# JianCao92/speaker-diarization

Hardware: AMD Instinct MI355X
Metric: diarized audio throughput (CD gw/BIC + CL hi/BIC) (higher is better)
Workload: dtype f64

## Files before the change

speaker-diarization_amd/csrc/spkd_cluster.hpp:

```cpp
#pragma once
#include "spkd_device.hpp"
#include "spkd_quad.hpp"
#include "spkd_tri.hpp"
#include "../../include/spkd.h"

namespace spkd {

constexpr double MAXINT_F = 9223372036854775808.0;
constexpr double PEN_UNIT = 39.0 + 0.5 * 39.0 * 40.0;
constexpr int AUX = 3 * DA;
constexpr int ERR_DEGENERATE_MERGE = 2;

__device__ __forceinline__ unsigned long long dkey(double v) {
    unsigned long long b = (unsigned long long)__double_as_longlong(v);
    return (b >> 63) ? ~b : (b | 0x8000000000000000ull);
}
__device__ __forceinline__ double dkey_inv(unsigned long long k) {
    unsigned long long b = (k >> 63) ? (k & 0x7fffffffffffffffull) : ~k;
    return __longlong_as_double((long long)b);
}
template <bool MAXOP>
__device__ __forceinline__ unsigned wave_red_u32(unsigned x) {
    auto op = [](unsigned a, unsigned b) { return MAXOP ? (a > b ? a : b) : (a < b ? a : b); };
    x = op(x, (unsigned)__builtin_amdgcn_update_dpp((int)x, (int)x, 0xB1, 0xf, 0xf, false));
// ... 556 lines not shown
    r.mc = okey != ~0ull ? (int)oc : NO_COL;
    r.nc = __any(nc != NO_COL) ? (int)wave_red_u32<false>((unsigned)nc) : NO_COL;
    return r;
}

__device__ __forceinline__ bool row_cache_after_merge(int variant, double d, int sa, int sb,
                                                      double& rm, int& ra, int& rn) {
    if (variant != 1) return ra == sb || rn == sb;
    const bool nan_hit = rn == sa || rn == sb;
    if (ra == sa || ra == sb || nan_hit) {
        if (nan_hit || !(d < rm)) return true;
        rm = d; ra = sa;
    } else if (d != d) {
        if (sa < rn) rn = sa;
    } else if (d < rm || (d == rm && sa < ra)) {
        rm = d; ra = sa;
    }
    return false;
}

template <class Alive>
__device__ __forceinline__ double final_matrix_max(const double* __restrict__ Dm, long long N, Alive alive,
                                                   double* s_tmax, int tid) {
    const int lane = tid & (WAVE - 1), wave = tid >> 6;
    double tmax = -__builtin_huge_val();
    bool anynan = false;
    for (long long r = wave; r < N; r += AHC_WAVES) {
        if (!alive(r)) continue;
        const double* row = Dm + r * N;
        for (long long c = lane; c < N; c += WAVE) {
            if (!alive(c)) continue;
            const double v = row[c];
            if (v != v) anynan = true; else tmax = v > tmax ? v : tmax;
        }
    }
#pragma unroll
    for (int s = 1; s < WAVE; s <<= 1) {
        const double t2 = __shfl_xor(tmax, s);
        tmax = t2 > tmax ? t2 : tmax;
    }
    anynan = __any(anynan);
    if (lane == 0) s_tmax[wave] = anynan ? __builtin_nan("") : tmax;
    __syncthreads();
    double mx = s_tmax[0];
    if (tid == 0) {
        for (int w = 1; w < AHC_WAVES; ++w) {
            const double x = s_tmax[w];
            if (mx == mx) mx = (x != x) ? x : (x > mx ? x : mx);
        }
    }
    return mx;
}

__device__ __forceinline__ void refresh_rows(const double* __restrict__ Dm, long long N,
                                             const int32_t* __restrict__ al, int32_t* __restrict__ dirty,
                                             double* __restrict__ rmin, int32_t* __restrict__ rarg,
                                             int32_t* __restrict__ rnan, unsigned long long* masks,
                                             int tid, int wave, int lane) {
    const long long n_chunks = (N + WAVE - 1) / WAVE;
    for (long long ch = wave; ch < n_chunks; ch += AHC_WAVES) {
        const long long rl = ch * WAVE + lane;
        const long long rc = rl < N ? rl : N - 1;
        const int fa = al[rc], fd = dirty[rc];
        const unsigned long long mk = __ballot(rl < N && fa && fd);
        if (lane == 0) masks[ch] = mk;
    }
    __syncthreads();
    int ord = 0;
    for (long long ch = 0; ch < n_chunks; ++ch) {
        const long long r0 = ch * WAVE;
        unsigned long long todo = masks[ch];
        while (todo) {
            const int b = __builtin_ctzll(todo);
            todo &= todo - 1;
            if ((ord++ & (AHC_WAVES - 1)) != wave) continue;
            const long long r = r0 + b;
            const RowMin e = scan_row(Dm + r * N, N, [&](long long c) { return al[c] != 0; }, -1, 0.0, lane);
            if (lane == 0) { rmin[r] = e.mv; rarg[r] = e.mc; rnan[r] = e.nc; dirty[r] = 0; }
#ifdef SPKD_PROFILE
            if (lane == 0) atomicAdd(&g_ahc_prof[0], 1ull);
#endif
        }
    }
}

template <bool TWO>
__global__ __launch_bounds__(AHC_TPB) void k_ahc(
        double* __restrict__ ex, double* __restrict__ pk, const int64_t* __restrict__ seg_off,
        int variant, int kind, int max_spk, double lambdac, double threshold,
        double* __restrict__ ld, double* __restrict__ aux,
        double* __restrict__ mat, const int64_t* __restrict__ mat_off,
        int32_t* __restrict__ alive, double* __restrict__ tmp,
        double* __restrict__ rmin_all, int32_t* __restrict__ rcache_all,
        int32_t* __restrict__ out_n, int32_t* __restrict__ out_a, int32_t* __restrict__ out_b,
        double* __restrict__ out_d, unsigned long long* stat_max, unsigned long long* stat_min,
        double* __restrict__ final_max, double* __restrict__ final_min, int* err,
        double* pinv_ws) {
    extern __shared__ int32_t ids[];
    __shared__ double ldsA[QREC];
    __shared__ unsigned long long red3[AHC_WAVES][3];
    __shared__ unsigned long long s_masks[AHC_MAX_N / WAVE];
    __shared__ int s_cnt[2];
    __shared__ int s_nids;
    __shared__ int s_next;
    __shared__ double s_tmax[AHC_WAVES];
    const int tid = threadIdx.x, lane = lane_id(), wave = tid >> 6;
    const QuadLane L = quad_lane();
    const int p = blockIdx.x;
    const int64_t off = seg_off[p];
    const long long N = seg_off[p + 1] - off;
    double* Dm = mat + mat_off[p];
    int32_t* al = alive + off;
    double* ldp = ld + off;
    double* tp = tmp + off;
    double* rmin = rmin_all + off;
    int32_t* rarg = rcache_all + 3 * off;
    int32_t* rnan = rarg + N;
    int32_t* dirty = rnan + N;
    for (long long c = tid; c < N; c += AHC_TPB) { al[c] = 1; dirty[c] = 1; }
    __syncthreads();
    long long m = N;
    int n_merges = 0;
    const long long INF_IDX = 0x7fffffffffffffffLL;
    double fmin = 0.0;
#ifdef SPKD_PROFILE
    unsigned long long ahc_acc[5] = {0ull, 0ull, 0ull, 0ull, 0ull}, ahc_t = clock64();
#define AHC_TICK(i) do { const unsigned long long now_ = clock64(); ahc_acc[i] += now_ - ahc_t; ahc_t = now_; } while (0)
#else
#define AHC_TICK(i) ((void)0)
#endif
    while (true) {
        refresh_rows(Dm, N, al, dirty, rmin, rarg, rnan, s_masks, tid, wave, lane);
        __syncthreads();
        AHC_TICK(0);
        unsigned long long kb = ~0ull, ib = ~0ull, inan = ~0ull;
        for (long long r = tid; r < N; r += AHC_TPB) {
            if (!al[r]) continue;
            const double v = rmin[r];
            const int c = rarg[r], nc = rnan[r];
            if (nc != NO_COL) { const unsigned long long l = (unsigned long long)(r * N + nc); inan = l < inan ? l : inan; }
            if (c != NO_COL) {
                const unsigned long long kv = dkey(v);
                if (kv < kb) { kb = kv; ib = (unsigned long long)(r * N + c); }
            }
        }
        {
            const unsigned long long wk = wave_red_u64<false>(kb);
            const unsigned long long wi = wave_red_u64<false>(kb == wk ? ib : ~0ull);
            const unsigned long long wn = __any(inan != ~0ull) ? wave_red_u64<false>(inan) : ~0ull;
            if (lane == 0) { red3[wave][0] = wk; red3[wave][1] = wi; red3[wave][2] = wn; }
        }
        __syncthreads();
        unsigned long long bk = red3[0][0], bi = red3[0][1], bn = red3[0][2];
#pragma unroll
        for (int w = 1; w < AHC_WAVES; ++w) {
            const unsigned long long ok = red3[w][0], oi = red3[w][1], on = red3[w][2];
            const bool t = ok < bk || (ok == bk && oi < bi);
            bk = t ? ok : bk; bi = t ? oi : bi;
            bn = on < bn ? on : bn;
        }
        const bool has_nan = bn != ~0ull;
        const double mind = has_nan ? __builtin_nan("") : (bi != ~0ull ? dkey_inv(bk) : __builtin_huge_val());
        const long long index = has_nan ? (long long)bn : (bi != ~0ull ? (long long)bi : INF_IDX);
        fmin = mind;
        const bool go = (mind <= threshold) || (max_spk > 0 && m > max_spk);
        if (!go) break;
        AHC_TICK(1);
        const long long r0 = index / N, c0 = index - r0 * N;
        if (r0 == c0) {
            if (tid == 0) atomicOr(err, ERR_DEGENERATE_MERGE);
            break;
        }
        const long long sa = r0 < c0 ? r0 : c0, sb = r0 < c0 ? c0 : r0;
        if (tid < 2) s_cnt[tid] = 0;
        if (tid == 0) { s_nids = 1; s_next = 0; }
        __syncthreads();
        {
            int ca = 0, cb = 0;
            for (long long c = tid; c < sb; c += AHC_TPB) {
                if (al[c]) { cb++; if (c < sa) ca++; }
            }
            ca = __builtin_amdgcn_readlane(wave_scan_i32(ca), WAVE - 1);
            cb = __builtin_amdgcn_readlane(wave_scan_i32(cb), WAVE - 1);
            if (lane == 0 && ca) atomicAdd(&s_cnt[0], ca);
            if (lane == 0 && cb) atomicAdd(&s_cnt[1], cb);
        }
        __syncthreads();
        if (tid == 0) {
            const int64_t o = off + n_merges;
            out_a[o] = s_cnt[0]; out_b[o] = s_cnt[1]; out_d[o] = mind;
            al[sb] = 0;
            ids[0] = (int32_t)sa;
        }
        n_merges++;
        m--;
#ifdef SPKD_PROFILE
        if (tid == 0) atomicAdd(&g_ahc_prof[1], 1ull);
#endif
        double* A = ex + (off + sa) * QREC;
        const double* B = ex + (off + sb) * QREC;
        {
            double* Ap = pk + (off + sa) * REC;
            const double* Bp = pk + (off + sb) * REC;
            constexpr int NQ = (QREC + AHC_TPB - 1) / AHC_TPB, NP = (REC + AHC_TPB - 1) / AHC_TPB;
            double qa[NQ], qb[NQ], pa[NP], pb[NP];
#pragma unroll
            for (int u = 0; u < NQ; ++u) {
                const int e = tid + u * AHC_TPB;
                qa[u] = A[e < QREC ? e : 0]; qb[u] = B[e < QREC ? e : 0];
            }
#pragma unroll
            for (int u = 0; u < NP; ++u) {
                const int e = tid + u * AHC_TPB;
                pa[u] = Ap[e < REC ? e : 0]; pb[u] = Bp[e < REC ? e : 0];
            }
#pragma unroll
            for (int u = 0; u < NQ; ++u) {
                const int e = tid + u * AHC_TPB;
                const double v = qa[u] + qb[u];
                if (e < QREC) { A[e] = v; ldsA[e] = v; }
            }
#pragma unroll
            for (int u = 0; u < NP; ++u) {
                const int e = tid + u * AHC_TPB;
                if (e < REC) Ap[e] = pa[u] + pb[u];
            }
        }
        __syncthreads();
        for (long long c0 = 0; c0 < N; c0 += AHC_TPB) {
            const long long c = c0 + tid;
            const bool take = c < N && c != sa && al[c < N ? c : N - 1];
            const unsigned long long mk = __ballot(take);
            int base = 0;
            if (lane == 0 && mk) base = atomicAdd(&s_nids, __popcll(mk));
            base = __shfl(base, 0);
            if (take) ids[base + __popcll(mk & ((1ull << lane) - 1ull))] = (int32_t)c;
        }
        __syncthreads();
        AHC_TICK(2);
        const int nids = s_nids;
        const double nA = ldsA[QREC_COUNT_AT];
        if (kind == SPKD_KL2) {
            if (wave == 0) kl2_aux_from_qr(ldsA, aux + (off + sa) * AUX, pinv_ws);
        } else {
            for (;;) {
                int q4 = 0;
                if (lane == 0) q4 = atomicAdd(&s_next, 1);
                const int base = 4 * __builtin_amdgcn_readfirstlane(q4);
                if (base >= nids) break;
                int k = base + L.m;
                const bool valid = k < nids;
                k = valid ? k : nids - 1;
                const int32_t slot = ids[k];
                const double v = quad_pair_det<TWO>(kind, ldsA, nA, A, ex + (off + slot) * QREC, pk + (off + slot) * REC, k == 0, L, err);
                if (valid && L.t == 0) {
                    if (k == 0) ldp[sa] = log(v); else tp[slot] = v;
                }
            }
        }
        __syncthreads();
        AHC_TICK(3);
        double wmax = __builtin_nan(""), wmin = __builtin_nan("");
        const double ldA = ldp[sa];
        for (long long c = tid; c < N; c += AHC_TPB) {
            if (c == sa || !al[c]) continue;
            double d;
            if (kind == SPKD_KL2) {
                d = kl2_from_aux_serial(aux + (off + sa) * AUX, aux + (off + c) * AUX);
            } else {
                const double nC = qr_count(ex + (off + c) * QREC);
                d = finish_distance(kind, lambdac, nA, ldA, nC, ldp[c], log(tp[c]));
            }
            Dm[sa * N + c] = d;
            const double rm0 = rmin[c];
            const int ra0 = rarg[c], rn0 = rnan[c];
            double rm = rm0;
            int ra = ra0, rn = rn0;
            if (variant == 1) Dm[c * N + sa] = d;
            if (row_cache_after_merge(variant, d, (int)sa, (int)sb, rm, ra, rn)) dirty[c] = 1;
            else {
                if (rm != rm0 || ra != ra0) { rmin[c] = rm; rarg[c] = ra; }
                if (rn != rn0) rnan[c] = rn;
            }
            if (variant == 1 && stat_valid(d)) {
                wmax = (wmax != wmax || d > wmax) ? d : wmax;
                wmin = (wmin != wmin || d < wmin) ? d : wmin;
            }
        }
        if (tid == 0) dirty[sa] = 1;
        if (variant == 1) {
            const unsigned long long kmax = wave_red_u64<true>(wmax == wmax ? dkey(wmax) : 0ull);
            const unsigned long long kmin = wave_red_u64<false>(wmin == wmin ? dkey(wmin) : ~0ull);
            if (lane == 0) {
                if (kmax != 0ull) atomicMax(stat_max + p, kmax);
                if (kmin != ~0ull) atomicMin(stat_min + p, kmin);
            }
        }
        __syncthreads();
        AHC_TICK(4);
    }
#ifdef SPKD_PROFILE
    if (tid == 0) for (int i = 0; i < 5; ++i) atomicAdd(&g_ahc_prof[2 + i], ahc_acc[i]);
#endif
    const double mx = final_matrix_max(Dm, N, [&](long long c) { return al[c] != 0; }, s_tmax, tid);
    if (tid == 0) {
        out_n[p] = n_merges;
        final_max[p] = mx;
        final_min[p] = fmin;
    }
}

constexpr int STEP_WAVES = 4;
constexpr int STEP_WIDE_FROM = 1024;
constexpr int STEP_PARTNERS = 4 * STEP_WAVES - 1;
constexpr int ALIVE_ROUND = 0x7fffffff;
constexpr int STEP_MAX_N = 16384;
constexpr int STEP_IDX_SHIFT = 14;

struct StepState {
    int32_t done, n_merges;
    long long psa;
    double fmin;
    double diag;
};

__host__ __device__ inline unsigned long long step_slot_word(int round, int new_slot, int old_slot) {
    return ((unsigned long long)(unsigned)round << 40) | ((unsigned long long)(unsigned)new_slot << 20) |
           (unsigned long long)(unsigned)old_slot;
}
__device__ __forceinline__ int step_slot_of(unsigned long long w, int k) {
    return ((int)(w >> 40) < k) ? (int)((w >> 20) & 0xfffffull) : (int)(w & 0xfffffull);
}

struct StepSel {
    double rmin, newrow;
    int32_t rarg, rnan, death, pad;
};

struct StepArrays {
    double* ex;
    double* pk;
    double* exm;
    double* pkm;
    int32_t* death;
    StepSel* sel2;
    unsigned long long* sw;
    double* cnt;
    StepState* state2;
    int64_t n_total;
    int32_t n_prob;
};

__global__ __launch_bounds__(AHC_TPB) void k_step_init(
        const int64_t* __restrict__ seg_off, const double* __restrict__ mat,
        const int64_t* __restrict__ mat_off, StepArrays Q) {
    const int lane = lane_id(), wave = threadIdx.x >> 6;
    const int p = blockIdx.y;
    const int64_t off = seg_off[p];
    const long long N = seg_off[p + 1] - off;
    if (blockIdx.x == 0 && threadIdx.x == 0) {
        StepState S;
// ... 312 lines not shown
    if (kind != SPKD_KL2 && lead && tid == 0) ldp[sa] = ldA;
    {
        const int j = tid;
        bool rescan = false;
        double d = 0.0;
        if (fin) {
            const long long r = fin_r;
            if (kind == SPKD_KL2) d = kl2_from_aux_serial(s_auxA, aux + (off + r) * AUX);
            else d = finish_distance(kind, lambdac, nA, ldA, fin_nC, fin_ld, s_ldx[j]);
            double rm;
            int ra, rn;
            if (r == psa) { rm = s_psa.mv; ra = s_psa.mc; rn = s_psa.nc; }
            else { rm = fin_sel.rmin; ra = fin_sel.rarg; rn = fin_sel.rnan; }
            Dm[sa * N + r] = d;
            sel_w[r].newrow = d;
            if (variant == 1) Dm[r * N + sa] = d;
            rescan = row_cache_after_merge(variant, d, (int)sa, (int)sb, rm, ra, rn);
            if (!rescan) { sel_w[r].rmin = rm; sel_w[r].rarg = ra; sel_w[r].rnan = rn; }
        }
        if (tid < 4 * STEP_WAVES) { s_rescan[tid] = rescan ? 1 : 0; s_dfin[tid] = d; }
        __syncthreads();
        for (int jj = 1 + wave; jj <= mine_n; jj += SW) {
            if (!s_rescan[jj]) continue;
            const long long r = s_ids[first + jj - 1];
            const RowMin e = scan_row(Dm + r * N, N, [&](long long c) { return c != sb && death[c] > k; },
                                      variant == 1 ? sa : -1, s_dfin[jj], lane);
            if (lane == 0) { sel_w[r].rmin = e.mv; sel_w[r].rarg = e.mc; sel_w[r].rnan = e.nc; }
        }
    }
    STEP_TICK(6);
#ifdef SPKD_PROFILE
    if (lead && tid == 0) atomicAdd(&g_ahc_prof[1], 1ull);
#endif
    if (lead && tid == 0) {
        StepState T;
        T.done = 0; T.n_merges = n_merges + 1; T.psa = sa; T.fmin = mind; T.diag = diag_sa;
        *Snext = T;
    }
}

__global__ __launch_bounds__(AHC_TPB) void k_step_final(
        int last_round, const int64_t* __restrict__ seg_off, const double* __restrict__ mat,
        const int64_t* __restrict__ mat_off, StepArrays Q, int32_t* __restrict__ out_n,
        double* __restrict__ final_max, double* __restrict__ final_min) {
    __shared__ double s_tmax[AHC_WAVES];
    const int tid = threadIdx.x;
    const int p = blockIdx.x;
    const int64_t off = seg_off[p];
    const long long N = seg_off[p + 1] - off;
    const int32_t* death = Q.death + off;
    const StepState S = Q.state2[(size_t)((last_round + 1) & 1) * Q.n_prob + p];
    const double mx = final_matrix_max(mat + mat_off[p], N, [&](long long c) { return death[c] == ALIVE_ROUND; }, s_tmax, tid);
    if (tid == 0) {
        out_n[p] = S.n_merges;
        final_max[p] = mx;
        final_min[p] = S.fmin;
    }
}

constexpr int CIN_WAVES = 4;
constexpr int CIN_TPB = CIN_WAVES * WAVE;

struct CinKeep {
    double* dist;
    long long cap;
    long long* dist_off;
    int* status;
    long long off = 0;
    __device__ bool room(long long K) const { return off + K <= cap; }
    __device__ void refuse() const { atomicOr(status, 4); }
    __device__ double* row() const { return dist + off; }
    __device__ void step() {}
    __device__ void seen(double) {}
    __device__ void decided(long long s, long long K, double, bool lead) {
        off += K;
        if (lead) dist_off[s + 1] = off;
    }
};

struct CinSummary {
    double* dists;
    double* mind;
    double smax = __builtin_nan(""), smin = __builtin_nan("");
    double tmax = __builtin_nan(""), tmin = __builtin_nan("");
    __device__ bool room(long long) const { return true; }
    __device__ void refuse() const {}
    __device__ double* row() const { return dists; }
    __device__ void step() { tmax = tmin = __builtin_nan(""); }
    __device__ void seen(double d) {
        if (!stat_valid(d)) return;
        if (!(tmax >= d)) tmax = d;
        if (!(tmin <= d)) tmin = d;
    }
    __device__ void decided(long long s, long long, double m, bool lead) {
        if (!lead) return;
        mind[s] = m;
        if (tmax == tmax && !(smax >= tmax)) smax = tmax;
        if (tmin == tmin && !(smin <= tmin)) smin = tmin;
    }
};

template <bool TWO, class Out>
__device__ __forceinline__ long long cluster_in_chain(
        const double* __restrict__ seg_ex, const double* __restrict__ seg_pk, const double* __restrict__ seg_ld,
        const double* __restrict__ seg_aux, long long n, int kind, double lambdac, double threshold,
        double* __restrict__ clu_ex, double* __restrict__ clu_pk, double* __restrict__ clu_ld, double* __restrict__ clu_aux,
        double* __restrict__ tmp, int32_t* __restrict__ label, Out& out, long long& K, int* err,
        double* pinv_ws) {
    __shared__ double ldsA[QREC];
// ... 140 lines not shown
```

speaker-diarization_amd/csrc/spkd_hip.hip:

```cpp
#include <hip/hip_runtime.h>

#include <algorithm>
#include <cmath>
#include <cstddef>
#include <cstdio>
#include <cstdlib>
#include <cstring>
#include <string>
#include <atomic>
#include <thread>
#include <vector>

#include "../../include/spkd.h"
#include "spkd_cd.hpp"
#include "spkd_cluster.hpp"
#include "spkd_device.hpp"
#include "spkd_handoff.hpp"
#include "spkd_stats.hpp"
#include "spkd_mfcc.hpp"
#include "spkd_vad.hpp"

using namespace spkd;

namespace {
constexpr int N_SLOTS = 40;
enum { PIN_GW_TURNS = 0, PIN_GW_LINES, PIN_AHC_OUT, N_PIN };
}

struct spkd_ctx {
    int device = 0;
    hipStream_t stream = nullptr;
    bool own_stream = false;
    bool gw_lds_ok = false;
    int gw_waves = 0;
    unsigned long long init_keys[2] = {0ull, ~0ull};
    int step_waves = 0;
    int step_partners = 0;
    int64_t last_gw_items = 0;
    std::string err;
    int* d_err = nullptr;
    unsigned long long* d_counter = nullptr;
    hipEvent_t ev0 = nullptr, ev1 = nullptr;
    float last_ms = 0.f;
    hipEvent_t ka[SPKD_N_TIMERS] = {}, kb[SPKD_N_TIMERS] = {};
    bool kused[SPKD_N_TIMERS] = {};
    float kms[SPKD_N_TIMERS] = {};
    void* slot[N_SLOTS] = {};
    size_t slot_bytes[N_SLOTS] = {};
    void* pinv_ws = nullptr;
    double* pinv_cur = nullptr;
    void* pin[N_PIN] = {};
    size_t pin_bytes[N_PIN] = {};
    std::vector<int64_t> redo_line, redo_begin, redo_end;
    std::vector<Chunk> redo_chunks;
    std::vector<int64_t> redo_setoff;
    std::vector<int32_t> redo_sets;
};

namespace {

spkd_status fail(spkd_ctx* c, spkd_status s, const std::string& msg) {
    if (c) c->err = msg;
    return s;
}

#define HIPCHK(c, call)                                                              \
    do {                                                                             \
        hipError_t e_ = (call);                                                      \
        if (e_ != hipSuccess)                                                        \
            return fail((c), SPKD_EHIP, std::string(#call) + ": " + hipGetErrorString(e_)); \
    } while (0)

#define TRY(expr) do { const spkd_status s_ = (expr); if (s_ != SPKD_OK) return s_; } while (0)

spkd_status scratch(spkd_ctx* c, int slot, size_t bytes, void** out) {
    if (bytes == 0) bytes = 16;
    if (c->slot_bytes[slot] < bytes) {
        if (c->slot[slot]) HIPCHK(c, hipFree(c->slot[slot]));
        c->slot[slot] = nullptr;
        c->slot_bytes[slot] = 0;
        size_t want = bytes + bytes / 4;
        hipError_t e = hipMalloc(&c->slot[slot], want);
        if (e != hipSuccess) {
            want = bytes;
            e = hipMalloc(&c->slot[slot], want);
        }
        if (e != hipSuccess) return fail(c, SPKD_ENOMEM, "scratch allocation failed");
        c->slot_bytes[slot] = want;
    }
    *out = c->slot[slot];
// ... 122 lines not shown
    spkd_ctx* const c;
    const int idx;
    Timer(spkd_ctx* ctx, int i) : c(ctx), idx(i) { (void)hipEventRecord(c->ka[idx], c->stream); }
    ~Timer() { (void)hipEventRecord(c->kb[idx], c->stream); c->kused[idx] = true; }
};

enum {
    S_CHUNKS = 0, S_SETOFF, S_PARTIAL, S_IDXA, S_IDXB, S_TERMS, S_TURNS, S_SNAP, S_CAND,
    S_GW_N_WIN, S_GW_WIN_DET, S_GW_WIN_MAXD, S_GW_DET_START, S_GW_DET_MAXI, S_GW_DET_D, S_GW_FINAL_START, S_LOG,
    S_AHC_STATS, S_AHC_LD, S_AHC_AUX, S_AHC_MAT, S_AHC_MISC, S_AHC_OUT, S_AHC_OFF, S_AHC_PROB, S_AHC_PACKED, S_MFCC_TAB, S_MFCC_STATIC,
    S_STEP_EXM, S_STEP_PKM, S_STEP_MISC, S_GMM_TAB, S_GMM_IDX,
    S_CP_TURNS, S_CP_TIMES, S_CP_LINES, S_REDO_STATS, S_REDO_IDX, S_COUNT
};
static_assert(S_COUNT <= N_SLOTS, "scratch slot table too small");

}

extern "C" {

int spkd_abi_version(void) { return SPKD_ABI_VERSION; }

static spkd_status create_ctx(int device, void* stream, bool borrow, spkd_ctx** out) {
    if (!out) return SPKD_EINVAL;
    *out = nullptr;
    int count = 0;
    if (hipGetDeviceCount(&count) != hipSuccess || device < 0 || device >= count) return SPKD_EHIP;
    spkd_ctx* c = new spkd_ctx();
    c->device = device;
    if (hipSetDevice(device) != hipSuccess) { delete c; return SPKD_EHIP; }
    if (borrow) {
        c->stream = (hipStream_t)stream;
    } else {
        if (hipStreamCreateWithFlags(&c->stream, hipStreamDefault) != hipSuccess) { delete c; return SPKD_EHIP; }
        c->own_stream = true;
    }
    if (hipMalloc(&c->d_err, sizeof(int)) != hipSuccess ||
        hipMalloc(&c->d_counter, 2 * sizeof(unsigned long long)) != hipSuccess ||
        hipEventCreate(&c->ev0) != hipSuccess || hipEventCreate(&c->ev1) != hipSuccess) {
        spkd_destroy(c);
        return SPKD_EHIP;
    }
    for (int i = 0; i < SPKD_N_TIMERS; ++i)
        if (hipEventCreate(&c->ka[i]) != hipSuccess || hipEventCreate(&c->kb[i]) != hipSuccess) {
            spkd_destroy(c);
            return SPKD_EHIP;
        }
    int lds_max = 0;
    c->gw_lds_ok = hipDeviceGetAttribute(&lds_max, hipDeviceAttributeMaxSharedMemoryPerBlock, device) == hipSuccess &&
                   Gw<4>::LDS_BYTES <= lds_max &&
                   hipFuncSetAttribute((const void*)k_gw<8>, hipFuncAttributeMaxDynamicSharedMemorySize, Gw<8>::LDS_BYTES) == hipSuccess &&
                   hipFuncSetAttribute((const void*)k_gw<4>, hipFuncAttributeMaxDynamicSharedMemorySize, Gw<4>::LDS_BYTES) == hipSuccess &&
                   hipFuncSetAttribute((const void*)k_gw<2>, hipFuncAttributeMaxDynamicSharedMemorySize, Gw<2>::LDS_BYTES) == hipSuccess &&
                   hipFuncSetAttribute((const void*)k_gw<1>, hipFuncAttributeMaxDynamicSharedMemorySize, Gw<1>::LDS_BYTES) == hipSuccess;
    if (const char* e = getenv("SPKD_GW_WAVES")) c->gw_waves = atoi(e);
    if (const char* e = getenv("SPKD_STEP_WAVES")) { const int v = atoi(e); c->step_waves = (v == 4 || v == 8) ? v : 0; }
    if (const char* e = getenv("SPKD_STEP_PARTNERS")) { const int v = atoi(e); c->step_partners = (v == 3 || v == 7 || v == 15) ? v : 0; }
    *out = c;
    return SPKD_OK;
}

spkd_status spkd_create(int device, void* stream, spkd_ctx** out) {
    return create_ctx(device, stream, stream != nullptr, out);
}

spkd_status spkd_create_on_stream(int device, void* stream, spkd_ctx** out) {
    return create_ctx(device, stream, true, out);
}

void spkd_destroy(spkd_ctx* c) {
    if (!c) return;
    (void)hipSetDevice(c->device);
    if (c->stream) (void)hipStreamSynchronize(c->stream);
    for (int i = 0; i < N_SLOTS; ++i)
        if (c->slot[i]) (void)hipFree(c->slot[i]);
    if (c->d_err) (void)hipFree(c->d_err);
    if (c->pinv_ws) (void)hipFree(c->pinv_ws);
    for (int i = 0; i < N_PIN; ++i)
        if (c->pin[i]) (void)hipHostFree(c->pin[i]);
    if (c->d_counter) (void)hipFree(c->d_counter);
    if (c->ev0) (void)hipEventDestroy(c->ev0);
    if (c->ev1) (void)hipEventDestroy(c->ev1);
    for (int i = 0; i < SPKD_N_TIMERS; ++i) {
        if (c->ka[i]) (void)hipEventDestroy(c->ka[i]);
        if (c->kb[i]) (void)hipEventDestroy(c->kb[i]);
    }
    if (c->own_stream && c->stream) (void)hipStreamDestroy(c->stream);
    delete c;
}

const char* spkd_last_error(const spkd_ctx* c) { return c ? c->err.c_str() : "null context"; }

spkd_status spkd_sync(spkd_ctx* c) {
    if (!c) return SPKD_EINVAL;
    HIPCHK(c, hipStreamSynchronize(c->stream));
    return SPKD_OK;
}

spkd_status spkd_malloc(spkd_ctx* c, size_t bytes, void** d_ptr) {
    if (!c || !d_ptr) return SPKD_EINVAL;
    HIPCHK(c, hipSetDevice(c->device));
    hipError_t e = hipMalloc(d_ptr, bytes ? bytes : 16);
    if (e != hipSuccess) return fail(c, SPKD_ENOMEM, hipGetErrorString(e));
    return SPKD_OK;
}

spkd_status spkd_free(spkd_ctx* c, void* d_ptr) {
// ... 434 lines not shown
        h_n_done[p] = done2[2 * p];
        h_n_clusters[p] = done2[2 * p + 1];
    }
    return st;
}

spkd_status spkd_distance_rows(spkd_ctx* c, int variant, int kind, double lambdac, const double* d_stats,
                               int64_t n, int64_t row_begin, int64_t row_end, double* d_rows,
                               double* h_stat_max, double* h_stat_min) {
    if (!c || n < 0 || bad_kind(kind) || (variant != 1 && variant != 2)) return SPKD_EINVAL;
    if (row_begin < 0 || row_end < row_begin || row_end > n) return fail(c, SPKD_EINVAL, "distance_rows: bad row block");
    if (h_stat_max) *h_stat_max = std::nan("");
    if (h_stat_min) *h_stat_min = std::nan("");
    if (n == 0 || row_end == row_begin) return SPKD_OK;
    if (!d_stats || !d_rows) return fail(c, SPKD_EINVAL, "null argument");
    const int64_t seg_off[2] = {0, n};
    AhcPrep B;
    MatrixPlan plan;
    plan.row_begin = row_begin;
    plan.row_end = row_end;
    unsigned long long keys[2] = {0ull, ~0ull};
    Call call(c);
    TRY(call.opened);
    TRY(use_kind(c, kind, &kind));
    TRY(ahc_prepare(c, d_stats, seg_off, 1, variant, kind, lambdac, B, plan));
    HIPCHK(c, hipMemcpyAsync(d_rows, B.mat + row_begin * n, (size_t)(row_end - row_begin) * n * sizeof(double),
                             hipMemcpyDeviceToDevice, c->stream));
    HIPCHK(c, hipMemcpyAsync(&keys[0], B.smax, sizeof(unsigned long long), hipMemcpyDeviceToHost, c->stream));
    HIPCHK(c, hipMemcpyAsync(&keys[1], B.smin, sizeof(unsigned long long), hipMemcpyDeviceToHost, c->stream));
    const spkd_status st = call.finish();
    if (h_stat_max) *h_stat_max = key_to_double(keys[0], true);
    if (h_stat_min) *h_stat_min = key_to_double(keys[1], false);
    return st;
}

namespace {
spkd_status ahc_impl(spkd_ctx* c, const double* d_stats, const int64_t* h_seg_off, int64_t n_prob,
                     const spkd_ahc_params* P, const MatrixPlan& plan, int32_t* h_n_merges, int32_t* h_merge_a,
                     int32_t* h_merge_b, double* h_merge_d, double* h_stat_max, double* h_stat_min) {
    if (!c || !P || n_prob < 0) return SPKD_EINVAL;
    if (n_prob == 0) return SPKD_OK;
    if (!d_stats || !h_seg_off || !h_n_merges || !h_merge_a || !h_merge_b || !h_merge_d ||
        !h_stat_max || !h_stat_min)
        return fail(c, SPKD_EINVAL, "null argument");
    if ((P->variant != 1 && P->variant != 2) || bad_kind(P->kind))
        return fail(c, SPKD_EINVAL, "bad variant / kind");
    for (int64_t p = 0; p < n_prob; ++p)
        if (h_seg_off[p + 1] - h_seg_off[p] < 1) return fail(c, SPKD_EINVAL, "empty clustering problem");
    int64_t n_max = 0;
    for (int64_t p = 0; p < n_prob; ++p) n_max = std::max<int64_t>(n_max, h_seg_off[p + 1] - h_seg_off[p]);
    if (n_max > AHC_MAX_N) return fail(c, SPKD_EINVAL, "clustering problem larger than 65536 records");
    int path = P->path;
    if (path != SPKD_AHC_MONO && path != SPKD_AHC_WIDE) path = n_prob <= 64 ? SPKD_AHC_WIDE : SPKD_AHC_MONO;
    const size_t lds = (size_t)(n_max + 4) * sizeof(int32_t);
    if (path == SPKD_AHC_MONO && lds > 150 * 1024) path = SPKD_AHC_WIDE;
    if (path == SPKD_AHC_WIDE && n_max > STEP_MAX_N)
        return fail(c, SPKD_EINVAL, "clustering problem larger than 16384 records (wide merge loop)");
    AhcPrep B;
    std::vector<unsigned long long> kmax((size_t)n_prob), kmin((size_t)n_prob);
    std::vector<double> fmax((size_t)n_prob), fmin((size_t)n_prob);
    Call call(c);
    TRY(call.opened);
    spkd_ahc_params Pk;
    TRY(kernel_params(c, P, Pk));
    TRY(ahc_prepare(c, d_stats, h_seg_off, n_prob, P->variant, P->kind, P->lambdac, B, plan));
    const int64_t n_total = B.n_total;
    const size_t nt = (size_t)n_total, np = (size_t)n_prob;
    double *d_merge_d, *d_tmp, *d_rmin, *d_fmax, *d_fmin;
    int32_t *d_a, *d_b, *d_alive, *d_rcache, *d_n;
    TRY(carve(c, scratch, S_AHC_OUT, [&](Layout L) {
        return L.part(d_merge_d, nt).part(d_tmp, nt).part(d_rmin, nt).part(d_fmax, np).part(d_fmin, np)
            .part(d_a, nt).part(d_b, nt).part(d_alive, nt).part(d_rcache, 3 * nt).part(d_n, np).bytes();
    }));
    if (path == SPKD_AHC_MONO) {
        auto kahc = P->kind == SPKD_GLR ? k_ahc<true> : k_ahc<false>;
        if (lds > 48 * 1024)
            (void)hipFuncSetAttribute((const void*)kahc, hipFuncAttributeMaxDynamicSharedMemorySize, (int)lds);
        Timer t(c, SPKD_T_AHC);
        hipLaunchKernelGGL(kahc, dim3((unsigned)n_prob), dim3(AHC_TPB), lds, c->stream,
                           B.ex, B.pk, (const int64_t*)B.seg_off, P->variant, P->kind, P->max_spk, P->lambdac,
                           P->threshold, B.ld, B.aux, B.mat, (const int64_t*)B.mat_off, d_alive, d_tmp,
                           d_rmin, d_rcache, d_n, d_a, d_b, d_merge_d, B.smax, B.smin, d_fmax, d_fmin, c->d_err,
                           c->pinv_cur);
    } else {
        StepArrays Q;
        void *pe = nullptr, *pp = nullptr;
        TRY(carve(c, scratch, S_STEP_MISC, [&](Layout L) {
            return L.part(Q.sel2, 2 * nt).part(Q.cnt, nt).part(Q.sw, nt).part(Q.state2, 2 * np).part(Q.death, nt).bytes();
        }));
        TRY(scratch(c, S_STEP_EXM, nt * QREC * sizeof(double), &pe));
        TRY(scratch(c, S_STEP_PKM, nt * REC * sizeof(double), &pp));
        Q.ex = B.ex; Q.pk = B.pk; Q.exm = (double*)pe; Q.pkm = (double*)pp;
        Q.n_total = n_total;
        Q.n_prob = (int32_t)n_prob;
        const int step_waves = c->step_waves ? c->step_waves : (n_max > STEP_WIDE_FROM ? 8 : 4);
        const bool glr_k = P->kind == SPKD_GLR;
        using StepKernel = decltype(&k_ahc_step<false, 4, 3>);
        StepKernel kvar[3];
        if (step_waves == 8) {
            kvar[0] = glr_k ? k_ahc_step<true, 8, 3> : k_ahc_step<false, 8, 3>;
            kvar[1] = glr_k ? k_ahc_step<true, 8, 7> : k_ahc_step<false, 8, 7>;
            kvar[2] = glr_k ? k_ahc_step<true, 8, STEP_PARTNERS> : k_ahc_step<false, 8, STEP_PARTNERS>;
        } else {
            kvar[0] = glr_k ? k_ahc_step<true, 4, 3> : k_ahc_step<false, 4, 3>;
            kvar[1] = glr_k ? k_ahc_step<true, 4, 7> : k_ahc_step<false, 4, 7>;
            kvar[2] = glr_k ? k_ahc_step<true, 4, STEP_PARTNERS> : k_ahc_step<false, 4, STEP_PARTNERS>;
        }
        auto sp_of_round = [&](int64_t partners) -> int {
            if (c->step_partners) return c->step_partners;
            const int64_t free_cus = 255;
            if (partners * n_prob <= 3 * free_cus) return 3;
            if (partners * n_prob <= 7 * free_cus) return 7;
            return STEP_PARTNERS;
        };
        const size_t nch_max = (size_t)((n_max + WAVE - 1) / WAVE);
        const size_t step_lds = ((size_t)2 * n_max + nch_max + 2) * sizeof(int32_t) + nch_max * sizeof(unsigned long long);
        if (step_lds + 20 * 1024 > 48 * 1024)
            for (int v = 0; v < 3; ++v)
                (void)hipFuncSetAttribute((const void*)kvar[v], hipFuncAttributeMaxDynamicSharedMemorySize, (int)step_lds);
        Timer t(c, SPKD_T_AHC);
        const unsigned row_blocks = (unsigned)((n_max + AHC_WAVES - 1) / AHC_WAVES);
        hipLaunchKernelGGL(k_step_init, dim3(row_blocks, (unsigned)n_prob), dim3(AHC_TPB), 0, c->stream,
                           (const int64_t*)B.seg_off, (const double*)B.mat, (const int64_t*)B.mat_off, Q);
        for (int64_t it = 1; it < n_max; ++it) {
            const int64_t partners = n_max - it - 1;
            const int step_sp = sp_of_round(partners);
            StepKernel kstep = kvar[step_sp == 3 ? 0 : (step_sp == 7 ? 1 : 2)];
            const unsigned blocks = (unsigned)std::max<int64_t>(1, (partners + step_sp - 1) / step_sp) + 1;
            hipLaunchKernelGGL(kstep, dim3(blocks, (unsigned)n_prob), dim3(step_waves * WAVE), step_lds, c->stream,
                               (int)it, (const int64_t*)B.seg_off, P->variant, P->kind, P->max_spk, P->lambdac,
                               P->threshold, B.ld, B.aux, B.mat, (const int64_t*)B.mat_off, Q, d_a, d_b, d_merge_d,
                               B.smax, B.smin, c->d_err, c->pinv_cur);
        }
        hipLaunchKernelGGL(k_step_final, dim3((unsigned)n_prob), dim3(AHC_TPB), 0, c->stream,
                           (int)(n_max - 1), (const int64_t*)B.seg_off, (const double*)B.mat, (const int64_t*)B.mat_off,
// ... 1042 lines not shown
```

Measured before the change: 1422.

## Keep per-cluster AHC state in LDS and fuse merge bookkeeping passes

Moves the per-row AHC state (alive flags, row-min cache, log-dets, tmp, counts) into dynamic LDS when a clustering problem fits, falling back to global memory for large ones. It also folds the alive-count and id-compaction passes into the merge update and builds the dirty-row masks directly with ballots during the distance update, dropping the separate dirty array and its mask-building pass and some barriers. The larger LDS footprint can lower occupancy, and a final_min fix is added to the wide path.

```diff
diff --git a/speaker-diarization_amd/csrc/spkd_cluster.hpp b/speaker-diarization_amd/csrc/spkd_cluster.hpp
--- a/speaker-diarization_amd/csrc/spkd_cluster.hpp
+++ b/speaker-diarization_amd/csrc/spkd_cluster.hpp
@@ -632,20 +632,21 @@
     return mx;
 }
 
-__device__ __forceinline__ void refresh_rows(const double* __restrict__ Dm, long long N,
-                                             const int32_t* __restrict__ al, int32_t* __restrict__ dirty,
-                                             double* __restrict__ rmin, int32_t* __restrict__ rarg,
-                                             int32_t* __restrict__ rnan, unsigned long long* masks,
-                                             int tid, int wave, int lane) {
+struct AhcState {
+    int32_t *alive, *rarg, *rnan;
+    double *rmin, *ld, *tmp, *cnt;
+};
+constexpr int AHC_LDS_MAX_N = 2560;
+__host__ __device__ constexpr size_t ahc_ids_ints(long long n) { return (size_t)((n + 2) & ~1LL); }
+__host__ __device__ constexpr size_t ahc_lds_bytes(long long n_state, long long n_ids) {
+    const size_t ids_only = ahc_ids_ints(n_ids) * sizeof(int32_t);
+    const size_t with_state = ahc_ids_ints(n_state) * sizeof(int32_t) + (size_t)n_state * (4 * sizeof(double) + 3 * sizeof(int32_t));
+    return n_state > 0 && with_state > ids_only ? with_state : ids_only;
+}
+
+__device__ __forceinline__ void refresh_rows(const double* __restrict__ Dm, long long N, const AhcState S,
+                                             const unsigned long long* masks, int wave, int lane) {
     const long long n_chunks = (N + WAVE - 1) / WAVE;
-    for (long long ch = wave; ch < n_chunks; ch += AHC_WAVES) {
-        const long long rl = ch * WAVE + lane;
-        const long long rc = rl < N ? rl : N - 1;
-        const int fa = al[rc], fd = dirty[rc];
-        const unsigned long long mk = __ballot(rl < N && fa && fd);
-        if (lane == 0) masks[ch] = mk;
-    }
-    __syncthreads();
     int ord = 0;
     for (long long ch = 0; ch < n_chunks; ++ch) {
         const long long r0 = ch * WAVE;
@@ -655,8 +656,8 @@
             todo &= todo - 1;
             if ((ord++ & (AHC_WAVES - 1)) != wave) continue;
             const long long r = r0 + b;
-            const RowMin e = scan_row(Dm + r * N, N, [&](long long c) { return al[c] != 0; }, -1, 0.0, lane);
-            if (lane == 0) { rmin[r] = e.mv; rarg[r] = e.mc; rnan[r] = e.nc; dirty[r] = 0; }
+            const RowMin e = scan_row(Dm + r * N, N, [&](long long c) { return S.alive[c] != 0; }, -1, 0.0, lane);
+            if (lane == 0) { S.rmin[r] = e.mv; S.rarg[r] = e.mc; S.rnan[r] = e.nc; }
 #ifdef SPKD_PROFILE
             if (lane == 0) atomicAdd(&g_ahc_prof[0], 1ull);
 #endif
@@ -665,18 +666,15 @@
 }
 
 template <bool TWO>
-__global__ __launch_bounds__(AHC_TPB) void k_ahc(
-        double* __restrict__ ex, double* __restrict__ pk, const int64_t* __restrict__ seg_off,
+__device__ __forceinline__ void ahc_merge_loop(
+        const AhcState S, int32_t* ids, const int p, const int64_t off, const long long N,
+        double* __restrict__ ex, double* __restrict__ pk, const double* ld_prep,
         int variant, int kind, int max_spk, double lambdac, double threshold,
-        double* __restrict__ ld, double* __restrict__ aux,
-        double* __restrict__ mat, const int64_t* __restrict__ mat_off,
-        int32_t* __restrict__ alive, double* __restrict__ tmp,
-        double* __restrict__ rmin_all, int32_t* __restrict__ rcache_all,
+        double* __restrict__ aux, double* __restrict__ Dm,
         int32_t* __restrict__ out_n, int32_t* __restrict__ out_a, int32_t* __restrict__ out_b,
         double* __restrict__ out_d, unsigned long long* stat_max, unsigned long long* stat_min,
         double* __restrict__ final_max, double* __restrict__ final_min, int* err,
         double* pinv_ws) {
-    extern __shared__ int32_t ids[];
     __shared__ double ldsA[QREC];
     __shared__ unsigned long long red3[AHC_WAVES][3];
     __shared__ unsigned long long s_masks[AHC_MAX_N / WAVE];
@@ -686,18 +684,17 @@
     __shared__ double s_tmax[AHC_WAVES];
     const int tid = threadIdx.x, lane = lane_id(), wave = tid >> 6;
     const QuadLane L = quad_lane();
-    const int p = blockIdx.x;
-    const int64_t off = seg_off[p];
-    const long long N = seg_off[p + 1] - off;
-    double* Dm = mat + mat_off[p];
-    int32_t* al = alive + off;
-    double* ldp = ld + off;
-    double* tp = tmp + off;
-    double* rmin = rmin_all + off;
-    int32_t* rarg = rcache_all + 3 * off;
-    int32_t* rnan = rarg + N;
-    int32_t* dirty = rnan + N;
-    for (long long c = tid; c < N; c += AHC_TPB) { al[c] = 1; dirty[c] = 1; }
+    const long long n_chunks = (N + WAVE - 1) / WAVE;
+    for (long long c = tid; c < N; c += AHC_TPB) {
+        S.alive[c] = 1;
+        S.ld[c] = ld_prep[c];
+        S.cnt[c] = pk[(off + c) * REC + REC - 1];
+    }
+    for (long long ch = tid; ch < n_chunks; ch += AHC_TPB) {
+        const long long rows = N - ch * WAVE;
+        s_masks[ch] = rows >= WAVE ? ~0ull : (1ull << rows) - 1ull;
+    }
+    if (tid == 0) { s_cnt[0] = 0; s_cnt[1] = 0; s_nids = 1; s_next = 0; }
     __syncthreads();
     long long m = N;
     int n_merges = 0;
@@ -710,14 +707,14 @@
 #define AHC_TICK(i) ((void)0)
 #endif
     while (true) {
-        refresh_rows(Dm, N, al, dirty, rmin, rarg, rnan, s_masks, tid, wave, lane);
+        refresh_rows(Dm, N, S, s_masks, wave, lane);
         __syncthreads();
         AHC_TICK(0);
         unsigned long long kb = ~0ull, ib = ~0ull, inan = ~0ull;
         for (long long r = tid; r < N; r += AHC_TPB) {
-            if (!al[r]) continue;
-            const double v = rmin[r];
-            const int c = rarg[r], nc = rnan[r];
+            if (!S.alive[r]) continue;
+            const double v = S.rmin[r];
+            const int c = S.rarg[r], nc = S.rnan[r];
             if (nc != NO_COL) { const unsigned long long l = (unsigned long long)(r * N + nc); inan = l < inan ? l : inan; }
             if (c != NO_COL) {
                 const unsigned long long kv = dkey(v);
@@ -752,31 +749,6 @@
             break;
         }
         const long long sa = r0 < c0 ? r0 : c0, sb = r0 < c0 ? c0 : r0;
-        if (tid < 2) s_cnt[tid] = 0;
-        if (tid == 0) { s_nids = 1; s_next = 0; }
-        __syncthreads();
-        {
-            int ca = 0, cb = 0;
-            for (long long c = tid; c < sb; c += AHC_TPB) {
-                if (al[c]) { cb++; if (c < sa) ca++; }
-            }
-            ca = __builtin_amdgcn_readlane(wave_scan_i32(ca), WAVE - 1);
-            cb = __builtin_amdgcn_readlane(wave_scan_i32(cb), WAVE - 1);
-            if (lane == 0 && ca) atomicAdd(&s_cnt[0], ca);
-            if (lane == 0 && cb) atomicAdd(&s_cnt[1], cb);
-        }
-        __syncthreads();
-        if (tid == 0) {
-            const int64_t o = off + n_merges;
-            out_a[o] = s_cnt[0]; out_b[o] = s_cnt[1]; out_d[o] = mind;
-            al[sb] = 0;
-            ids[0] = (int32_t)sa;
-        }
-        n_merges++;
-        m--;
-#ifdef SPKD_PROFILE
-        if (tid == 0) atomicAdd(&g_ahc_prof[1], 1ull);
-#endif
         double* A = ex + (off + sa) * QREC;
         const double* B = ex + (off + sb) * QREC;
         {
@@ -794,11 +766,29 @@
                 const int e = tid + u * AHC_TPB;
                 pa[u] = Ap[e < REC ? e : 0]; pb[u] = Bp[e < REC ? e : 0];
             }
+            int ca = 0, cb = 0;
+            for (long long cw = 0; cw < N; cw += AHC_TPB) {
+                const long long c = cw + tid;
+                const bool a = c < N && S.alive[c < N ? c : N - 1];
+                if (a && c < sb) { cb++; if (c < sa) ca++; }
+                const bool take = a && c != sa && c != sb;
+                const unsigned long long mk = __ballot(take);
+                int base = 0;
+                if (lane == 0 && mk) base = atomicAdd(&s_nids, __popcll(mk));
+                base = __shfl(base, 0);
+                if (take) ids[base + __popcll(mk & ((1ull << lane) - 1ull))] = (int32_t)c;
+            }
+            ca = __builtin_amdgcn_readlane(wave_scan_i32(ca), WAVE - 1);
+            cb = __builtin_amdgcn_readlane(wave_scan_i32(cb), WAVE - 1);
+            if (lane == 0 && ca) atomicAdd(&s_cnt[0], ca);
+            if (lane == 0 && cb) atomicAdd(&s_cnt[1], cb);
+            if (tid == 0) ids[0] = (int32_t)sa;
 #pragma unroll
             for (int u = 0; u < NQ; ++u) {
                 const int e = tid + u * AHC_TPB;
                 const double v = qa[u] + qb[u];
                 if (e < QREC) { A[e] = v; ldsA[e] = v; }
+                if (e == QREC_COUNT_AT) S.cnt[sa] = v;
             }
 #pragma unroll
             for (int u = 0; u < NP; ++u) {
@@ -807,16 +797,16 @@
             }
         }
         __syncthreads();
-        for (long long c0 = 0; c0 < N; c0 += AHC_TPB) {
-            const long long c = c0 + tid;
-            const bool take = c < N && c != sa && al[c < N ? c : N - 1];
-            const unsigned long long mk = __ballot(take);
-            int base = 0;
-            if (lane == 0 && mk) base = atomicAdd(&s_nids, __popcll(mk));
-            base = __shfl(base, 0);
-            if (take) ids[base + __popcll(mk & ((1ull << lane) - 1ull))] = (int32_t)c;
-        }
-        __syncthreads();
+        if (tid == 0) {
+            const int64_t o = off + n_merges;
+            out_a[o] = s_cnt[0]; out_b[o] = s_cnt[1]; out_d[o] = mind;
+            S.alive[sb] = 0;
+        }
+        n_merges++;
+        m--;
+#ifdef SPKD_PROFILE
+        if (tid == 0) atomicAdd(&g_ahc_prof[1], 1ull);
+#endif
         AHC_TICK(2);
         const int nids = s_nids;
         const double nA = ldsA[QREC_COUNT_AT];
@@ -834,40 +824,45 @@
                 const int32_t slot = ids[k];
                 const double v = quad_pair_det<TWO>(kind, ldsA, nA, A, ex + (off + slot) * QREC, pk + (off + slot) * REC, k == 0, L, err);
                 if (valid && L.t == 0) {
-                    if (k == 0) ldp[sa] = log(v); else tp[slot] = v;
+                    if (k == 0) S.ld[sa] = log(v); else S.tmp[slot] = v;
                 }
             }
         }
         __syncthreads();
         AHC_TICK(3);
+        if (tid == 0) { s_cnt[0] = 0; s_cnt[1] = 0; s_nids = 1; s_next = 0; }
         double wmax = __builtin_nan(""), wmin = __builtin_nan("");
-        const double ldA = ldp[sa];
-        for (long long c = tid; c < N; c += AHC_TPB) {
-            if (c == sa || !al[c]) continue;
-            double d;
-            if (kind == SPKD_KL2) {
-                d = kl2_from_aux_serial(aux + (off + sa) * AUX, aux + (off + c) * AUX);
-            } else {
-                const double nC = qr_count(ex + (off + c) * QREC);
-                d = finish_distance(kind, lambdac, nA, ldA, nC, ldp[c], log(tp[c]));
-            }
-            Dm[sa * N + c] = d;
-            const double rm0 = rmin[c];
-            const int ra0 = rarg[c], rn0 = rnan[c];
-            double rm = rm0;
-            int ra = ra0, rn = rn0;
-            if (variant == 1) Dm[c * N + sa] = d;
-            if (row_cache_after_merge(variant, d, (int)sa, (int)sb, rm, ra, rn)) dirty[c] = 1;
-            else {
-                if (rm != rm0 || ra != ra0) { rmin[c] = rm; rarg[c] = ra; }
-                if (rn != rn0) rnan[c] = rn;
-            }
-            if (variant == 1 && stat_valid(d)) {
-                wmax = (wmax != wmax || d > wmax) ? d : wmax;
-                wmin = (wmin != wmin || d < wmin) ? d : wmin;
-            }
-        }
-        if (tid == 0) dirty[sa] = 1;
+        const double ldA = S.ld[sa];
+        for (long long cw = 0; cw < N; cw += AHC_TPB) {
+            const long long c = cw + tid;
+            bool redo = c == sa;
+            if (c < N && c != sa && S.alive[c]) {
+                double d;
+                if (kind == SPKD_KL2) {
+                    d = kl2_from_aux_serial(aux + (off + sa) * AUX, aux + (off + c) * AUX);
+                } else {
+                    d = finish_distance(kind, lambdac, nA, ldA, S.cnt[c], S.ld[c], log(S.tmp[c]));
+                }
+                Dm[sa * N + c] = d;
+                const double rm0 = S.rmin[c];
+                const int ra0 = S.rarg[c], rn0 = S.rnan[c];
+                double rm = rm0;
+                int ra = ra0, rn = rn0;
+                if (variant == 1) Dm[c * N + sa] = d;
+                redo = row_cache_after_merge(variant, d, (int)sa, (int)sb, rm, ra, rn);
+                if (!redo) {
+                    if (rm != rm0 || ra != ra0) { S.rmin[c] = rm; S.rarg[c] = ra; }
+                    if (rn != rn0) S.rnan[c] = rn;
+                }
+                if (variant == 1 && stat_valid(d)) {
+                    wmax = (wmax != wmax || d > wmax) ? d : wmax;
+                    wmin = (wmin != wmin || d < wmin) ? d : wmin;
+                }
+            }
+            const unsigned long long mk = __ballot(redo);
+            const long long ch = (cw >> 6) + wave;
+            if (lane == 0 && ch < n_chunks) s_masks[ch] = mk;
+        }
         if (variant == 1) {
             const unsigned long long kmax = wave_red_u64<true>(wmax == wmax ? dkey(wmax) : 0ull);
             const unsigned long long kmin = wave_red_u64<false>(wmin == wmin ? dkey(wmin) : ~0ull);
@@ -882,11 +877,44 @@
 #ifdef SPKD_PROFILE
     if (tid == 0) for (int i = 0; i < 5; ++i) atomicAdd(&g_ahc_prof[2 + i], ahc_acc[i]);
 #endif
-    const double mx = final_matrix_max(Dm, N, [&](long long c) { return al[c] != 0; }, s_tmax, tid);
+    const double mx = final_matrix_max(Dm, N, [&](long long c) { return S.alive[c] != 0; }, s_tmax, tid);
     if (tid == 0) {
         out_n[p] = n_merges;
         final_max[p] = mx;
         final_min[p] = fmin;
+    }
+}
+
+template <bool TWO>
+__global__ __launch_bounds__(AHC_TPB) void k_ahc(
+        double* __restrict__ ex, double* __restrict__ pk, const int64_t* __restrict__ seg_off,
+        int variant, int kind, int max_spk, double lambdac, double threshold,
+        double* __restrict__ ld, double* __restrict__ aux,
+        double* __restrict__ mat, const int64_t* __restrict__ mat_off, int lds_max_n,
+        int32_t* __restrict__ alive, double* __restrict__ tmp, double* __restrict__ cnt,
+        double* __restrict__ rmin_all, int32_t* __restrict__ rcache_all,
+        int32_t* __restrict__ out_n, int32_t* __restrict__ out_a, int32_t* __restrict__ out_b,
+        double* __restrict__ out_d, unsigned long long* stat_max, unsigned long long* stat_min,
+        double* __restrict__ final_max, double* __restrict__ final_min, int* err,
+        double* pinv_ws) {
+    extern __shared__ int32_t ids[];
+    const int p = blockIdx.x;
+    const int64_t off = seg_off[p];
+    const long long N = seg_off[p + 1] - off;
+    double* Dm = mat + mat_off[p];
+    AhcState S;
+    if (N <= lds_max_n) {
+        double* d = reinterpret_cast<double*>(ids + ahc_ids_ints(N));
+        S.rmin = d; S.ld = d + N; S.tmp = d + 2 * N; S.cnt = d + 3 * N;
+        int32_t* w = reinterpret_cast<int32_t*>(d + 4 * N);
+        S.alive = w; S.rarg = w + N; S.rnan = w + 2 * N;
+        ahc_merge_loop<TWO>(S, ids, p, off, N, ex, pk, ld + off, variant, kind, max_spk, lambdac, threshold, aux, Dm,
+                            out_n, out_a, out_b, out_d, stat_max, stat_min, final_max, final_min, err, pinv_ws);
+    } else {
+        S.rmin = rmin_all + off; S.ld = ld + off; S.tmp = tmp + off; S.cnt = cnt + off;
+        S.alive = alive + off; S.rarg = rcache_all + 2 * off; S.rnan = S.rarg + N;
+        ahc_merge_loop<TWO>(S, ids, p, off, N, ex, pk, ld + off, variant, kind, max_spk, lambdac, threshold, aux, Dm,
+                            out_n, out_a, out_b, out_d, stat_max, stat_min, final_max, final_min, err, pinv_ws);
     }
 }
 
@@ -1305,9 +1333,13 @@
     const StepState S = Q.state2[(size_t)((last_round + 1) & 1) * Q.n_prob + p];
     const double mx = final_matrix_max(mat + mat_off[p], N, [&](long long c) { return death[c] == ALIVE_ROUND; }, s_tmax, tid);
     if (tid == 0) {
+        double fm = S.fmin;
+        if (!S.done && N > 1 && S.n_merges == N - 1)
+            for (long long c = 0; c < N; ++c)
+                if (death[c] == ALIVE_ROUND) fm = mat[mat_off[p] + c * N + c];
         out_n[p] = S.n_merges;
         final_max[p] = mx;
-        final_min[p] = S.fmin;
+        final_min[p] = fm;
     }
 }
 
diff --git a/speaker-diarization_amd/csrc/spkd_hip.hip b/speaker-diarization_amd/csrc/spkd_hip.hip
--- a/speaker-diarization_amd/csrc/spkd_hip.hip
+++ b/speaker-diarization_amd/csrc/spkd_hip.hip
@@ -36,6 +36,9 @@
     unsigned long long init_keys[2] = {0ull, ~0ull};
     int step_waves = 0;
     int step_partners = 0;
+    int ahc_lds_max_n = 0;
+    int ahc_lds_admit = 0;
+    bool ahc_lds_ok = false;
     int64_t last_gw_items = 0;
     std::string err;
     int* d_err = nullptr;
@@ -264,6 +267,23 @@
                    hipFuncSetAttribute((const void*)k_gw<4>, hipFuncAttributeMaxDynamicSharedMemorySize, Gw<4>::LDS_BYTES) == hipSuccess &&
                    hipFuncSetAttribute((const void*)k_gw<2>, hipFuncAttributeMaxDynamicSharedMemorySize, Gw<2>::LDS_BYTES) == hipSuccess &&
                    hipFuncSetAttribute((const void*)k_gw<1>, hipFuncAttributeMaxDynamicSharedMemorySize, Gw<1>::LDS_BYTES) == hipSuccess;
+    {
+        hipFuncAttributes fa;
+        size_t fixed = 0;
+        bool ok = true;
+        for (const void* k : {(const void*)k_ahc<false>, (const void*)k_ahc<true>}) {
+            ok = ok && hipFuncGetAttributes(&fa, k) == hipSuccess;
+            fixed = std::max(fixed, fa.sharedSizeBytes);
+        }
+        int64_t fit = ok && (size_t)lds_max > fixed + 8 ? (int64_t)(((size_t)lds_max - fixed - 8) / 48) : 0;
+        fit = std::min<int64_t>(fit, AHC_LDS_MAX_N);
+        c->ahc_lds_admit = (int)ahc_lds_bytes(fit, fit);
+        c->ahc_lds_ok = ok &&
+            hipFuncSetAttribute((const void*)k_ahc<false>, hipFuncAttributeMaxDynamicSharedMemorySize, c->ahc_lds_admit) == hipSuccess &&
+            hipFuncSetAttribute((const void*)k_ahc<true>, hipFuncAttributeMaxDynamicSharedMemorySize, c->ahc_lds_admit) == hipSuccess;
+        if (const char* e = getenv("SPKD_AHC_LDS_MAX_N")) fit = std::min<int64_t>(fit, std::max(0, atoi(e)));
+        c->ahc_lds_max_n = (int)fit;
+    }
     if (const char* e = getenv("SPKD_GW_WAVES")) c->gw_waves = atoi(e);
     if (const char* e = getenv("SPKD_STEP_WAVES")) { const int v = atoi(e); c->step_waves = (v == 4 || v == 8) ? v : 0; }
     if (const char* e = getenv("SPKD_STEP_PARTNERS")) { const int v = atoi(e); c->step_partners = (v == 3 || v == 7 || v == 15) ? v : 0; }
@@ -804,8 +824,13 @@
     if (n_max > AHC_MAX_N) return fail(c, SPKD_EINVAL, "clustering problem larger than 65536 records");
     int path = P->path;
     if (path != SPKD_AHC_MONO && path != SPKD_AHC_WIDE) path = n_prob <= 64 ? SPKD_AHC_WIDE : SPKD_AHC_MONO;
-    const size_t lds = (size_t)(n_max + 4) * sizeof(int32_t);
-    if (path == SPKD_AHC_MONO && lds > 150 * 1024) path = SPKD_AHC_WIDE;
+    int64_t n_lds = 0;
+    for (int64_t p = 0; p < n_prob; ++p) {
+        const int64_t n = h_seg_off[p + 1] - h_seg_off[p];
+        if (n <= c->ahc_lds_max_n) n_lds = std::max(n_lds, n);
+    }
+    const size_t lds = std::max(ahc_lds_bytes(n_lds, n_max), (size_t)(n_max + 4) * sizeof(int32_t));
+    if (path == SPKD_AHC_MONO && (size_t)(n_max + 4) * sizeof(int32_t) > 150 * 1024) path = SPKD_AHC_WIDE;
     if (path == SPKD_AHC_WIDE && n_max > STEP_MAX_N)
         return fail(c, SPKD_EINVAL, "clustering problem larger than 16384 records (wide merge loop)");
     AhcPrep B;
@@ -818,21 +843,22 @@
     TRY(ahc_prepare(c, d_stats, h_seg_off, n_prob, P->variant, P->kind, P->lambdac, B, plan));
     const int64_t n_total = B.n_total;
     const size_t nt = (size_t)n_total, np = (size_t)n_prob;
-    double *d_merge_d, *d_tmp, *d_rmin, *d_fmax, *d_fmin;
+    double *d_merge_d, *d_tmp, *d_cnt, *d_rmin, *d_fmax, *d_fmin;
     int32_t *d_a, *d_b, *d_alive, *d_rcache, *d_n;
     TRY(carve(c, scratch, S_AHC_OUT, [&](Layout L) {
-        return L.part(d_merge_d, nt).part(d_tmp, nt).part(d_rmin, nt).part(d_fmax, np).part(d_fmin, np)
-            .part(d_a, nt).part(d_b, nt).part(d_alive, nt).part(d_rcache, 3 * nt).part(d_n, np).bytes();
+        return L.part(d_merge_d, nt).part(d_tmp, nt).part(d_cnt, nt).part(d_rmin, nt).part(d_fmax, np).part(d_fmin, np)
+            .part(d_a, nt).part(d_b, nt).part(d_alive, nt).part(d_rcache, 2 * nt).part(d_n, np).bytes();
     }));
     if (path == SPKD_AHC_MONO) {
         auto kahc = P->kind == SPKD_GLR ? k_ahc<true> : k_ahc<false>;
-        if (lds > 48 * 1024)
+        if (!c->ahc_lds_ok) return fail(c, SPKD_EHIP, "k_ahc: dynamic LDS for the per-cluster state was not admitted");
+        if (lds > (size_t)c->ahc_lds_admit)
             (void)hipFuncSetAttribute((const void*)kahc, hipFuncAttributeMaxDynamicSharedMemorySize, (int)lds);
         Timer t(c, SPKD_T_AHC);
         hipLaunchKernelGGL(kahc, dim3((unsigned)n_prob), dim3(AHC_TPB), lds, c->stream,
                            B.ex, B.pk, (const int64_t*)B.seg_off, P->variant, P->kind, P->max_spk, P->lambdac,
-                           P->threshold, B.ld, B.aux, B.mat, (const int64_t*)B.mat_off, d_alive, d_tmp,
-                           d_rmin, d_rcache, d_n, d_a, d_b, d_merge_d, B.smax, B.smin, d_fmax, d_fmin, c->d_err,
+                           P->threshold, B.ld, B.aux, B.mat, (const int64_t*)B.mat_off, c->ahc_lds_max_n, d_alive, d_tmp,
+                           d_cnt, d_rmin, d_rcache, d_n, d_a, d_b, d_merge_d, B.smax, B.smin, d_fmax, d_fmin, c->d_err,
                            c->pinv_cur);
     } else {
         StepArrays Q;
```

Result: no change. 1435, median of 4 (+0.9%).
